# uniio/ivf-hnsw

Measured on AMD Instinct MI355X. Metric: queries/sec @ Recall@1, SIFT1B PQ16 nprobe=32; ADC scan HBM GB/s vs peak, higher is better.
Workload: dtype f32

## Files before the change

### ivf-hnsw_amd/csrc/device_common.h

```cpp
#pragma once
#include <hip/hip_runtime.h>
#include <stdint.h>

#include "scan_dispatch.h"

namespace ivfhnsw_gpu_impl {

__device__ __forceinline__ float l2_ref_order(const float *__restrict__ row, const float *sq, int d)
{
    float a0 = 0.f, a1 = 0.f, a2 = 0.f, a3 = 0.f, a4 = 0.f, a5 = 0.f, a6 = 0.f, a7 = 0.f;
    const float4 *r4 = reinterpret_cast<const float4 *>(row);
    const float4 *q4 = reinterpret_cast<const float4 *>(sq);
    for (int b = 0; b < d / 16; b++) {
        const float4 y0 = r4[4 * b], y1 = r4[4 * b + 1], y2 = r4[4 * b + 2], y3 = r4[4 * b + 3];
        const float4 x0 = q4[4 * b], x1 = q4[4 * b + 1], x2 = q4[4 * b + 2], x3 = q4[4 * b + 3];
        float t;
#define IVFHNSW_ACC(a, xv, yv) \
    t = __fsub_rn(xv, yv);     \
    a = __fadd_rn(a, __fmul_rn(t, t));
        IVFHNSW_ACC(a0, x0.x, y0.x) IVFHNSW_ACC(a1, x0.y, y0.y) IVFHNSW_ACC(a2, x0.z, y0.z) IVFHNSW_ACC(a3, x0.w, y0.w)
        IVFHNSW_ACC(a4, x1.x, y1.x) IVFHNSW_ACC(a5, x1.y, y1.y) IVFHNSW_ACC(a6, x1.z, y1.z) IVFHNSW_ACC(a7, x1.w, y1.w)
        IVFHNSW_ACC(a0, x2.x, y2.x) IVFHNSW_ACC(a1, x2.y, y2.y) IVFHNSW_ACC(a2, x2.z, y2.z) IVFHNSW_ACC(a3, x2.w, y2.w)
        IVFHNSW_ACC(a4, x3.x, y3.x) IVFHNSW_ACC(a5, x3.y, y3.y) IVFHNSW_ACC(a6, x3.z, y3.z) IVFHNSW_ACC(a7, x3.w, y3.w)
#undef IVFHNSW_ACC
// ... 126 lines not shown
        const float2 x = q2[4 * (j0 + i)];
        const float d0 = __fsub_rn(x.x, y[i].x), d1 = __fsub_rn(x.y, y[i].y);
        alo = __fadd_rn(alo, __fmul_rn(d0, d0));
        ahi = __fadd_rn(ahi, __fmul_rn(d1, d1));
    }
}

__device__ __forceinline__ float l2_ref_order_quad_batched(const float *row, const float *sq, int d, int t)
{
    const float2 *r2 = reinterpret_cast<const float2 *>(row) + t;
    const float2 *q2 = reinterpret_cast<const float2 *>(sq) + t;
    float alo = 0.f, ahi = 0.f;
    const int nj = d >> 3;
    int j0 = 0;
    for (; j0 + 16 <= nj; j0 += 16)
        l2_quad_block<16>(r2, q2, j0, alo, ahi);
    if (j0 + 8 <= nj) {
        l2_quad_block<8>(r2, q2, j0, alo, ahi);
        j0 += 8;
    }
    if (j0 + 4 <= nj) {
        l2_quad_block<4>(r2, q2, j0, alo, ahi);
        j0 += 4;
    }
    if (j0 + 2 <= nj)
        l2_quad_block<2>(r2, q2, j0, alo, ahi);
    float r = __fadd_rn(quad_bcast<0>(alo), quad_bcast<0>(ahi));
    r = __fadd_rn(r, quad_bcast<1>(alo));
    r = __fadd_rn(r, quad_bcast<1>(ahi));
    r = __fadd_rn(r, quad_bcast<2>(alo));
    r = __fadd_rn(r, quad_bcast<2>(ahi));
    r = __fadd_rn(r, quad_bcast<3>(alo));
    r = __fadd_rn(r, quad_bcast<3>(ahi));
    return r;
}

template <int NB>
__device__ __forceinline__ void l2_oct_block(const float *r1, const float *q1, int j0, float &acc)
{
    float y[NB];
#pragma unroll
    for (int i = 0; i < NB; i++)
        y[i] = r1[8 * (j0 + i)];
    asm volatile("" ::: "memory");
    __builtin_amdgcn_sched_barrier(0);
#pragma unroll
    for (int i = 0; i < NB; i++) {
        const float d0 = __fsub_rn(q1[8 * (j0 + i)], y[i]);
        acc = __fadd_rn(acc, __fmul_rn(d0, d0));
    }
}

__device__ __forceinline__ float l2_ref_order_oct(const float *row, const float *sq, int d, int t)
{
    const float *r1 = row + t;
    const float *q1 = sq + t;
    float acc = 0.f;
    const int nj = d >> 3;
    int j0 = 0;
    for (; j0 + 16 <= nj; j0 += 16)
        l2_oct_block<16>(r1, q1, j0, acc);
    if (j0 + 8 <= nj) {
        l2_oct_block<8>(r1, q1, j0, acc);
        j0 += 8;
    }
    if (j0 + 4 <= nj) {
        l2_oct_block<4>(r1, q1, j0, acc);
        j0 += 4;
    }
    if (j0 + 2 <= nj)
        l2_oct_block<2>(r1, q1, j0, acc);
    const float mir = __uint_as_float(
        (uint32_t)__builtin_amdgcn_update_dpp(0, (int)__float_as_uint(acc), 0x141, 0xf, 0xf, true));
    float r = __fadd_rn(quad_bcast<0>(acc), quad_bcast<1>(acc));
    r = __fadd_rn(r, quad_bcast<2>(acc));
    r = __fadd_rn(r, quad_bcast<3>(acc));
    r = __fadd_rn(r, quad_bcast<3>(mir));
    r = __fadd_rn(r, quad_bcast<2>(mir));
    r = __fadd_rn(r, quad_bcast<1>(mir));
    r = __fadd_rn(r, quad_bcast<0>(mir));
    return r;
}

template <int NJ>
__device__ __forceinline__ float l2_ref_order_oct_regs(const float *row, const float (&qr)[16], int t)
{
    const float *r1 = row + t;
    float y[NJ];
#pragma unroll
    for (int i = 0; i < NJ; i++)
        y[i] = r1[8 * i];
    asm volatile("" ::: "memory");
    __builtin_amdgcn_sched_barrier(0);
    float acc = 0.f;
#pragma unroll
    for (int i = 0; i < NJ; i++) {
        const float d0 = __fsub_rn(qr[i], y[i]);
        acc = __fadd_rn(acc, __fmul_rn(d0, d0));
    }
    const float mir = __uint_as_float(
        (uint32_t)__builtin_amdgcn_update_dpp(0, (int)__float_as_uint(acc), 0x141, 0xf, 0xf, true));
    float r = __fadd_rn(quad_bcast<0>(acc), quad_bcast<1>(acc));
    r = __fadd_rn(r, quad_bcast<2>(acc));
    r = __fadd_rn(r, quad_bcast<3>(acc));
    r = __fadd_rn(r, quad_bcast<3>(mir));
    r = __fadd_rn(r, quad_bcast<2>(mir));
    r = __fadd_rn(r, quad_bcast<1>(mir));
    r = __fadd_rn(r, quad_bcast<0>(mir));
    return r;
}

__device__ __forceinline__ float quad_sum8(float alo, float ahi)
{
    float r = __fadd_rn(quad_bcast<0>(alo), quad_bcast<0>(ahi));
    r = __fadd_rn(r, quad_bcast<1>(alo));
    r = __fadd_rn(r, quad_bcast<1>(ahi));
    r = __fadd_rn(r, quad_bcast<2>(alo));
    r = __fadd_rn(r, quad_bcast<2>(ahi));
    r = __fadd_rn(r, quad_bcast<3>(alo));
    r = __fadd_rn(r, quad_bcast<3>(ahi));
    return r;
}

__device__ __forceinline__ uint32_t wave_incl_scan(uint32_t v, int lane)
{
    (void)lane;
    int x = (int)v;
    x += __builtin_amdgcn_update_dpp(0, x, 0x111, 0xf, 0xf, true);
    x += __builtin_amdgcn_update_dpp(0, x, 0x112, 0xf, 0xf, true);
    x += __builtin_amdgcn_update_dpp(0, x, 0x114, 0xf, 0xf, true);
    x += __builtin_amdgcn_update_dpp(0, x, 0x118, 0xf, 0xf, true);
    x += __builtin_amdgcn_update_dpp(0, x, 0x142, 0xa, 0xf, false);
    x += __builtin_amdgcn_update_dpp(0, x, 0x143, 0xc, 0xf, false);
    return (uint32_t)x;
}

__device__ __forceinline__ unsigned long long wave_incl_scan_u64(unsigned long long v, int lane)
{
#pragma unroll
    for (int off = 1; off < 64; off <<= 1) {
        const unsigned long long o = __shfl_up(v, off, 64);
        if (lane >= off)
            v += o;
    }
    return v;
}

__device__ __forceinline__ uint64_t wave_min_u64(uint64_t v)
{
#pragma unroll
    for (int off = 32; off >= 1; off >>= 1) {
        uint64_t o = __shfl_xor((unsigned long long)v, off, 64);
        v = o < v ? o : v;
    }
    return v;
}

__device__ __forceinline__ uint32_t f32_orderable(float f)
{
    uint32_t u = __float_as_uint(f);
    return (u & 0x80000000u) ? ~u : (u | 0x80000000u);
}
__device__ __forceinline__ float orderable_f32(uint32_t o)
{
    return __uint_as_float((o & 0x80000000u) ? (o & 0x7fffffffu) : ~o);
}


template <int CS>
__device__ __forceinline__ void load_code_words(const uint8_t *__restrict__ codes, uint32_t gi, uint32_t (&w)[CS / 4])
{
    const uint8_t *p = codes + (size_t)gi * CS;
    if constexpr (CS % 16 == 0) {
#pragma unroll
        for (int i = 0; i < CS / 16; i++) {
            uint4 v = reinterpret_cast<const uint4 *>(p)[i];
            w[4 * i] = v.x, w[4 * i + 1] = v.y, w[4 * i + 2] = v.z, w[4 * i + 3] = v.w;
        }
    } else if constexpr (CS % 8 == 0) {
#pragma unroll
        for (int i = 0; i < CS / 8; i++) {
            uint2 v = reinterpret_cast<const uint2 *>(p)[i];
            w[2 * i] = v.x, w[2 * i + 1] = v.y;
        }
    } else {
#pragma unroll
        for (int i = 0; i < CS / 4; i++)
            w[i] = reinterpret_cast<const uint32_t *>(p)[i];
    }
}

template <int CS>
// ... 140 lines not shown
```

### ivf-hnsw_amd/csrc/kernels_hnsw.hip

```cpp
#include "ivfhnsw_kernels.h"
#include "device_common.h"
#include "walk_set.h"
#include "walk_shape.h"

#include <float.h>
#include <stdio.h>
#include <stdlib.h>
#include <type_traits>

namespace ivfhnsw_gpu_impl {

constexpr int vis_buckets(int minw, int tagw = 8)
{
    return minw <= 4 ? (tagw == 10 ? 1040 : 1008) : minw == 5 ? 768 : minw <= 7 ? 640 : 384;
}

template <int TAGW> struct VisFields {
    static constexpr int cntw = TAGW == 8 ? 8 : TAGW == 10 ? 14 : 16;
    static constexpr int cshift = 64 - cntw;
    static constexpr int slots = cshift / TAGW;
    static constexpr unsigned long long ones()
    {
        unsigned long long o = 0;
        for (int i = 0; i < slots; i++)
// ... 54 lines not shown
{
    static_assert(TAGW != 0, "LDS set only");
    constexpr unsigned long long kOnes = VisFields<TAGW>::ones();
    constexpr unsigned long long kHighs = kOnes << (TAGW - 1);
    const uint32_t b = id % (uint32_t)NB;
    const unsigned long long tag = (unsigned long long)((id / (uint32_t)NB) + 1);
    const unsigned long long old = vt[b];
    const unsigned long long x = old ^ (tag * kOnes);
    bucket_full = false;
    if ((x - kOnes) & ~x & kHighs)
        return true;
    bucket_full = (uint32_t)(old >> VisFields<TAGW>::cshift) >= (uint32_t)VisFields<TAGW>::slots;
    if (!bucket_full)
        return false;
    return (atomicOr(&bm[id >> 5], 0u) >> (id & 31)) & 1u;
}

__device__ __forceinline__ float byte_row_dist_half(const uint8_t *row, const float *sqp, int d, int h)
{
    const uint4 *r4 = reinterpret_cast<const uint4 *>(row);
    const int nchunk = d >> 4;
    float a0 = 0.f, a1 = 0.f, a2 = 0.f, a3 = 0.f;
    for (int j0 = h; j0 < nchunk; j0 += 8) {
        uint4 w[4];
#pragma unroll
        for (int i = 0; i < 4; i++)
            w[i] = j0 + 2 * i < nchunk ? r4[j0 + 2 * i] : make_uint4(0u, 0u, 0u, 0u);
        asm volatile("" ::: "memory");
        __builtin_amdgcn_sched_barrier(0);
#pragma unroll
        for (int i = 0; i < 4; i++) {
            if (j0 + 2 * i < nchunk) {
                const float4 *qq = reinterpret_cast<const float4 *>(sqp + 16 * (j0 + 2 * i));
                const uint32_t ws[4] = {w[i].x, w[i].y, w[i].z, w[i].w};
#pragma unroll
                for (int c = 0; c < 4; c++) {
                    const float4 qv = qq[c];
                    const float t0 = qv.x - (float)(ws[c] & 0xffu);
                    const float t1 = qv.y - (float)((ws[c] >> 8) & 0xffu);
                    const float t2 = qv.z - (float)((ws[c] >> 16) & 0xffu);
                    const float t3 = qv.w - (float)(ws[c] >> 24);
                    a0 = fmaf(t0, t0, a0);
                    a1 = fmaf(t1, t1, a1);
                    a2 = fmaf(t2, t2, a2);
                    a3 = fmaf(t3, t3, a3);
                }
            }
        }
    }
    return (a0 + a1) + (a2 + a3);
}

__device__ __forceinline__ unsigned long long walk_stamp()
{
    __builtin_amdgcn_sched_barrier(0);
    const unsigned long long t = __builtin_amdgcn_s_memtime();
    __builtin_amdgcn_s_waitcnt(0xC07F);
    __builtin_amdgcn_sched_barrier(0);
    return t;
}


struct WalkArgs {
    GraphTables g;
    const float *xq;
    int nq, nprobe, ef;
    uint32_t *coarse_ids;
    float *coarse_dists;
    uint32_t *visited;
    size_t vwords;
    uint32_t *status, *next_query, *redo_hdr, *redo_list;
    uint32_t *tail_bitmaps;
    unsigned long long *stamp_out;
};

template <class T> __device__ __forceinline__ const __attribute__((address_space(4))) T *late_kernarg()
{
    auto p = (const __attribute__((address_space(4))) T *)__builtin_amdgcn_kernarg_segment_ptr();
    asm volatile("" : "+s"(p));
    return p;
}

template <int NCH, int MINW, int TAGW, int FMODE, bool STAMPS = false, bool SPILL = false, int D = 0, int MAXM = 0,
          bool MERGE = true>
__global__ __launch_bounds__(64, MINW) void hnsw_walk_kernel(WalkArgs a)
{
    constexpr bool SHAPED = D != 0 && MAXM != 0;
    const GraphTables &g = a.g;
    const int ef = a.ef;
    uint32_t *__restrict__ const visited = a.visited;
    const size_t vwords = a.vwords;
#define WALK_COLD(f) (SHAPED ? late_kernarg<WalkArgs>()->f : a.f)
    extern __shared__ __attribute__((aligned(16))) unsigned char smem[];
    float *s_q = reinterpret_cast<float *>(smem);
    static_assert(!SHAPED || (FMODE >= 2 && !SPILL && MINW <= 4 && D % 16 == 0 && D <= 128 && MAXM <= 64),
                  "shape constants go with the neighbour-row forms");
    static_assert(SHAPED || MERGE, "the generic form reads merge_admissions at run time");
    const int dim = D ? D : g.d;
    const int maxm = MAXM ? MAXM : g.maxM;
    const int nbr_rows = MAXM ? (MAXM + 31) / 32 * 32 : g.nb_rows;
    float *s_qp = s_q + dim;
    const int dp = FMODE == 1 ? dim : 0;
    uint32_t *s_q8 = reinterpret_cast<uint32_t *>(s_qp + dp);
    unsigned long long *tail = reinterpret_cast<unsigned long long *>(smem + (size_t)(dim + dp) * sizeof(float) + 512);
    constexpr int NB = vis_buckets(MINW, TAGW);
    unsigned long long st_acc[9] = {0, 0, 0, 0, 0, 0}, st_t = 0;
    const int merge_extra = (NCH <= 4 && ef + 8 > kTailCap) ? ef + 8 - kTailCap : 0;
    unsigned long long *vt = tail + kTailCap + merge_extra;
    constexpr bool LDSVIS = TAGW != 0;

    const int lane = threadIdx.x;
    const int judged_row = 8 * (((lane >> 2) & 1) * 2 + (lane & 1)) + (lane >> 3);
    const bool merge_on = SHAPED ? MERGE : g.merge_admissions != 0;
    constexpr bool prefilter = FMODE != 0;
    constexpr bool inline_rows = FMODE >= 2;
    constexpr bool ROWNORMS = FMODE == 3;
    constexpr bool CK = FMODE >= 2;
    auto enc_id = [](uint32_t id, uint32_t c) { return CK ? (id << 7) | c : id; };
    auto dec_id = [](uint32_t e) { return CK ? e >> 7 : e; };
    uint32_t *bm = visited + (size_t)blockIdx.x * vwords;
    TailSpill spill;
    spill.bm = SPILL ? a.tail_bitmaps + (size_t)blockIdx.x * vwords : nullptr;
    spill.hi = -1;
    spill.count = 0;
    bool bitmap_dirty = !(LDSVIS && g.visited_clean);
    bool redo_ran = false;

    for (;;) {
        int q = 0;
        if constexpr (SPILL) {
            if (lane == 0) {
                const uint32_t i = atomicAdd(&a.redo_hdr[1], 1u);
                q = i < a.redo_hdr[0] ? (int)a.redo_list[i] : a.nq;
            }
        } else {
            if (lane == 0)
                q = (int)atomicAdd(WALK_COLD(next_query), 1u);
        }
        q = __builtin_amdgcn_readfirstlane(q);
        if (q >= WALK_COLD(nq))
            break;
        redo_ran = true;
        if (STAMPS)
            st_t = walk_stamp();

        if (!LDSVIS || bitmap_dirty) {
            uint4 *bm4 = reinterpret_cast<uint4 *>(bm);
            const size_t v4 = vwords / 4;
            for (size_t w = lane; w < v4; w += 64)
                bm4[w] = make_uint4(0u, 0u, 0u, 0u);
            bitmap_dirty = false;
        }
        if (LDSVIS)
            for (int w = lane; w < NB; w += 64)
                vt[w] = 0ull;
        __syncthreads();
        float qp_sq = 0.f;
        for (int i = lane; i < dim; i += 64) {
            const float v = WALK_COLD(xq)[(size_t)q * dim + i];
            s_q[i] = v;
            if (prefilter) {
                const float vp = __fdiv_rn(__fsub_rn(v, WALK_COLD(g.q_lo)), g.q_step);
                if (!inline_rows)
                    s_qp[i] = vp;
                qp_sq = fmaf(vp, vp, qp_sq);
            }
        }
        __syncthreads();
        constexpr bool QREG = MINW <= 4;
        float q_reg[QREG ? 16 : 1];
        if constexpr (QREG) {
#pragma unroll
            for (int i = 0; i < 16; i++)
                if constexpr (D != 0)
                    q_reg[i] = 8 * i < D ? s_q[8 * i + (lane & 7)] : 0.f;
                else
                    q_reg[i] = (g.d == 128 || g.d == 96) && 8 * i < g.d ? s_q[8 * i + (lane & 7)] : 0.f;
        }
        float pf_slack = 0.f, pf_slack_q = 0.f, pf_bonus = 0.f;
        int q16_w = 0;
        int x_const = 0;
        bool x_any = false;
        bool x_hi = false;
        uint4 qp_h = make_uint4(0u, 0u, 0u, 0u), qp_l = qp_h, qp_x = qp_h;
        if (prefilter) {
#pragma unroll
            for (int off = 32; off > 0; off >>= 1)
                qp_sq += __shfl_xor(qp_sq, off, 64);
            pf_slack = __uint_as_float(__builtin_amdgcn_readfirstlane(__float_as_uint(WALK_COLD(g.q_errc) + 3.9e-6f * sqrtf(qp_sq))));
// ... 254 lines not shown
                            if (x_hi) {
                                asm volatile("" ::);
#pragma unroll
                                for (int c = 0; c < 4; c++)
                                    xhr = __builtin_amdgcn_udot4(xh[c], ws[c], xhr, false);
                            }
                            X[i] = (int)(xlr - xhr);
                        }
                    }
                    int mine, minex = 0;
                    if (x_any)
                        oct_sum4x2(S, X, lane, mine, minex);
                    else
                        mine = oct_sum4(S, lane);
                    mine += (int)(128u * row_rr);
                    const float m1 = fmaxf(
                        0.f, __builtin_amdgcn_sqrtf((float)(mine + q16_w) * 0.0078125f) * 0.9990234375f - pf_slack_q);
                    const float m2 = fmaf(m1, m1, fmaf((float)(minex + x_const), 0.9990234375f, pf_bonus));
                    const float m = fmaxf(0.f, __builtin_amdgcn_sqrtf(m2) * 0.9990234375f - pf_slack) * g.q_step;
                    const float lb = m * m * 0.9990234375f;
                    const unsigned long long dropm = __ballot(lb > worst) & 0x3333333333333333ull;
                    const int rel = lane - rb;
                    const int ri = rel >> 3;
                    if (rel >= 0 && rel < 32 && ((dropm >> (8 * (rel & 7) + 4 * (ri >> 1) + (ri & 1))) & 1ull))
                        fresh = false;
                    rb += 32;
                    if (rb >= cnt)
                        break;
                    if constexpr (CK) {
                        const uint4 *nbr =
                            reinterpret_cast<const uint4 *>(g.nbrows + (size_t)node * nbr_rows * 128) + (lane & 7);
                        const int last = max(cnt - 1, 0);
#pragma unroll
                        for (int i = 0; i < 4; i++)
                            if (rb + 8 * i < cnt)
                                nw[i] = nbr[min(rb + 8 * i + (lane >> 3), last) * 8];
                    } else {
                        const uint4 *nbr =
                            reinterpret_cast<const uint4 *>(g.nbrows + ((size_t)node * nbr_rows + rb) * 128) + lane;
#pragma unroll
                        for (int i = 0; i < 4; i++)
                            nw[i] = nbr[i * 64];
                    }
                    if constexpr (ROWNORMS)
                        row_rr = g.nbnorms[(size_t)node * nbr_rows + rb + judged_row];
                }
                mask = __ballot(fresh);
                nfresh = __popcll(mask);
                if (filter_first) {
                    pend = fresh;
                    pend_full = full_now;
                    pend_id = nb;
                    pend_any = nfresh > 0;
                }
            } else if (filter_now && nfresh > 0) {
                const float worst = __uint_as_float(key_dist_bits(last_now));
                const int myrow = __popcll(mask & ((1ull << lane) - 1ull));
                for (int base = 0; base < nfresh; base += 32) {
                    const int r = base + (lane >> 1);
                    const bool active = r < nfresh;
                    const int src = active ? nth_set_bit(mask, r) : 0;
                    const uint32_t nbq = (uint32_t)__shfl((int)nb, src, 64);
                    float S = 0.f;
                    if (active)
                        S = byte_row_dist_half(g.qrows + (size_t)nbq * dim, s_qp, dim, lane & 1);
                    S += __shfl_xor(S, 1, 64);
                    const float m = fmaxf(0.f, __builtin_amdgcn_sqrtf(S) * 0.9990234375f - pf_slack) * g.q_step;
                    const float lb = m * m * 0.9990234375f;
                    const unsigned long long drop = __ballot(active && lb > worst);
                    const int rel = myrow - base;
                    if (fresh && rel >= 0 && rel < 32 && ((drop >> (2 * rel)) & 1ull))
                        fresh = false;
                }
                mask = __ballot(fresh);
                nfresh = __popcll(mask);
            }
            if (STAMPS) {
                const unsigned long long t = walk_stamp();
                st_acc[1] += t - st_t;
                st_t = t;
            }

            unsigned long long rest = mask;
            for (int base = 0; base < nfresh && ntail >= 0; base += 8) {
                const int r = base + (lane >> 3);
                const bool active = r < nfresh;
                const int src = take8_set_bits(rest, lane);
                const uint32_t nbe = (uint32_t)__shfl((int)nb_enc, src, 64);
                const uint32_t nbq = dec_id(nbe);
                float dq = 0.f;
                if (active) {
                    if constexpr (D != 0)
                        dq = l2_ref_order_oct_regs<D / 8>(g.vectors + (size_t)nbq * D, q_reg, lane & 7);
                    else if constexpr (QREG)
                        dq = g.d == 128  ? l2_ref_order_oct_regs<16>(g.vectors + (size_t)nbq * 128, q_reg, lane & 7)
                             : g.d == 96 ? l2_ref_order_oct_regs<12>(g.vectors + (size_t)nbq * 96, q_reg, lane & 7)
                                         : l2_ref_order_oct(g.vectors + (size_t)nbq * g.d, s_q, g.d, lane & 7);
                    else
                        dq = l2_ref_order_oct(g.vectors + (size_t)nbq * g.d, s_q, g.d, lane & 7);
                }
                if (STAMPS) {
                    asm volatile("s_waitcnt vmcnt(0)" ::: "memory");
                    const unsigned long long t = walk_stamp();
                    st_acc[2] += t - st_t;
                    st_t = t;
                }
                unsigned long long topk = base == 0 ? last_now : R.get(set_n() - 1);
                const float top0 = __uint_as_float(key_dist_bits(topk));
                unsigned long long cand = (!STEADY && n < ef ? ~0ull : __ballot(top0 > dq)) & 0x0101010101010101ull &
                                          lanes_below(8 * (nfresh - base), 0);
                if (STAMPS) {
                    st_acc[6] += (unsigned long long)__popcll(__ballot(active && (lane & 7) == 0));
                    st_acc[7] += (unsigned long long)__popcll(cand);
                }
                if (NCH <= 4 && merge_on && (STEADY || n == ef) && ntail == 0 && cand) {
                    const bool is_cand = (cand >> lane) & 1ull;
                    const unsigned long long Kc = mk_key(dq, nbe);
                    int dn[NCH];
#pragma unroll
                    for (int cc = 0; cc < NCH; cc++)
                        dn[cc] = 0;
                    const int ncand = __popcll(cand);
                    int cand_below = 0, set_below = 0;
                    for (unsigned long long cm = cand; cm; cm &= cm - 1) {
                        const int b = __ffsll((long long)cm) - 1;
                        const unsigned long long Kj = readlane_u64(Kc, b);
                        int below = 0;
#pragma unroll
                        for (int cc = 0; cc < NCH; cc++) {
                            const bool lt = (R.r[cc] & ~1ull) < Kj;
                            below += __popcll(__ballot(lt) & lanes_below(ef, cc));
                            dn[cc] += lt ? 1 : 0;
                        }
                        cand_below += Kj < Kc ? 1 : 0;
                        set_below = lane == b ? below : set_below;
                    }
                    unsigned long long *mb = tail;
#pragma unroll
                    for (int cc = 0; cc < NCH; cc++)
                        if (cc * 64 + lane < ef)
                            mb[cc * 64 + lane + (ncand - dn[cc])] = R.r[cc];
                    if (is_cand)
                        mb[set_below + cand_below] = Kc;
                    __syncthreads();
                    const unsigned long long b_lo = mb[ef - 1], b_hi = mb[ef];
                    unsigned long long merged[NCH];
#pragma unroll
                    for (int cc = 0; cc < NCH; cc++)
                        merged[cc] = cc * 64 + lane < ef ? mb[cc * 64 + lane] : R.r[cc];
                    const bool clean = key_dist_bits(b_lo) != key_dist_bits(b_hi);
                    if (clean) {
#pragma unroll
                        for (int cc = 0; cc < NCH; cc++)
                            R.r[cc] = merged[cc];
                        if (STAMPS)
                            st_acc[8] += (unsigned long long)__popcll(__ballot(is_cand && set_below + cand_below < ef));
                        cand = 0;
                    }
                    __syncthreads();
                }
                while (cand) {
                    const int b = __ffsll((long long)cand) - 1;
                    cand &= cand - 1;
                    const float dj = __uint_as_float((uint32_t)__builtin_amdgcn_readlane((int)__float_as_uint(dq), b));
                    const uint32_t idj = (uint32_t)__builtin_amdgcn_readlane((int)nbe, b);
                    const unsigned long long oldtop = topk;
                    if (!(__uint_as_float(key_dist_bits(oldtop)) > dj || (!STEADY && n < ef)))
                        continue;
                    const unsigned long long K = mk_key(dj, idj);
                    const bool full = STEADY || n == ef;
                    if (STAMPS)
                        st_acc[8] += 1;
                    R.insert_sorted(K, lane);
                    if (!full)
                        n++;
                    topk = R.get(set_n() - 1);
                    const uint32_t newmax = key_dist_bits(topk);
                    if (ntail > 0 && (SPILL ? tail_db : key_dist_bits(tail[0])) != newmax) {
                        ntail = 0;
                        if (SPILL && spill.count > 0)
                            spill.clear(lane);
                    }
                    if (full && !(oldtop & 1ull) && key_dist_bits(oldtop) == newmax) {
                        if (SPILL)
                            tail_db = newmax;
                        if ((!SPILL || spill.count == 0) && ntail < kTailCap) {
                            __syncthreads();
                            if (lane == 0)
                                tail[ntail] = oldtop;
                            ntail++;
                            __syncthreads();
                        } else if constexpr (SPILL) {
                            if (spill.count == 0) {
                                __syncthreads();
                                for (int t = 0; t < ntail; t++)
                                    spill.add(dec_id(key_id(tail[t])), lane);
                                __syncthreads();
                            }
                            spill.add(dec_id(key_id(oldtop)), lane);
                            ntail++;
                        } else {
                            if (lane == 0)
                                WALK_COLD(redo_list)[atomicAdd(&WALK_COLD(redo_hdr)[0], 1u)] = (uint32_t)q;
                            ntail = -1;
                            break;
                        }
                    }
                }
                if (STAMPS) {
                    const unsigned long long t = walk_stamp();
                    st_acc[3] += t - st_t;
                    st_t = t;
                }
            }
            return ntail >= 0;
        };
        if constexpr (SHAPED) {
            bool live = true;
            while (live && n < ef)
                live = expand(std::integral_constant<int, 1>{});
            while (live)
                live = expand(std::integral_constant<int, 2>{});
        } else {
            while (expand(std::integral_constant<int, 0>{})) {
            }
        }

        if (SPILL && spill.count > 0)
            spill.clear(lane);
        if (LDSVIS && __ballot(used_bitmap))
            bitmap_dirty = true;
        if (ntail >= 0) {
#pragma unroll
            for (int cc = 0; cc < NCH; cc++) {
                const int i = cc * 64 + lane;
                const int nprobe = WALK_COLD(nprobe);
                if (i < nprobe) {
                    const bool have = i < n;
                    WALK_COLD(coarse_ids)[(size_t)q * nprobe + i] = have ? dec_id(key_id(R.r[cc])) : 0xffffffffu;
                    WALK_COLD(coarse_dists)[(size_t)q * nprobe + i] = have ? __uint_as_float(key_dist_bits(R.r[cc])) : 0.f;
                }
            }
        }
    }
    if constexpr (SPILL) {
        if (lane == 0) {
            __threadfence();
            if (atomicAdd(&a.redo_hdr[2], 1u) == gridDim.x - 1) {
                a.redo_hdr[-1] = 0;
                a.redo_hdr[0] = 0;
                a.redo_hdr[1] = 0;
                a.redo_hdr[2] = 0;
            }
        }
    }
    if (SPILL && redo_ran) {
        uint4 *bm4 = reinterpret_cast<uint4 *>(bm);
        for (size_t w = lane; w < vwords / 4; w += 64)
            bm4[w] = make_uint4(0u, 0u, 0u, 0u);
    }
    if (LDSVIS && bitmap_dirty) {
        uint4 *bm4 = reinterpret_cast<uint4 *>(bm);
        for (size_t w = lane; w < vwords / 4; w += 64)
            bm4[w] = make_uint4(0u, 0u, 0u, 0u);
    }
    if (STAMPS && a.stamp_out && lane == 0)
        for (int i = 0; i < 9; i++)
            atomicAdd(&a.stamp_out[i], st_acc[i]);
#undef WALK_COLD
}

__global__ __launch_bounds__(64) void build_nbrows_kernel(GraphTables g, uint8_t *__restrict__ nbrows,
                                                          uint32_t *__restrict__ nbnorms, int nb_rows,
                                                          uint32_t *__restrict__ links_c)
{
    const size_t node = blockIdx.x;
    const int cnt = g.counts[node];
    if ((int)threadIdx.x < g.maxM) {
        uint32_t e = 0;
        if ((int)threadIdx.x < cnt) {
            const uint32_t id = g.links[node * g.maxM + threadIdx.x];
            e = id | ((uint32_t)g.counts[id] << 24);
        }
        links_c[node * g.maxM + threadIdx.x] = e;
    }
    const int cpr = g.d >> 4;
    for (int r0 = 0; r0 < nb_rows; r0 += 8) {
        const int r = r0 + (threadIdx.x >> 3), c = threadIdx.x & 7;
        uint4 v = make_uint4(0u, 0u, 0u, 0u);
        if (r < cnt && c < cpr)
            v = reinterpret_cast<const uint4 *>(g.qrows + (size_t)g.links[node * g.maxM + r] * g.d)[c];
        reinterpret_cast<uint4 *>(nbrows + (node * nb_rows + r) * 128)[c] = v;
        uint32_t rr = 0;
        rr = __builtin_amdgcn_udot4(v.x, v.x, rr, false);
        rr = __builtin_amdgcn_udot4(v.y, v.y, rr, false);
        rr = __builtin_amdgcn_udot4(v.z, v.z, rr, false);
        rr = __builtin_amdgcn_udot4(v.w, v.w, rr, false);
        rr = (uint32_t)oct_sum((int)rr);
        if (c == 0)
            nbnorms[node * nb_rows + r] = rr;
    }
}

hipError_t launch_build_nbrows(hipStream_t s, const GraphTables &g, uint8_t *nbrows, uint32_t *nbnorms, int nb_rows,
                               uint32_t *links_c)
{
    if (!g.qrows || g.d > 128 || (g.d & 15) || nb_rows < g.maxM || (nb_rows & 31) || g.n >= (1u << 24) || g.maxM > 64)
        return hipErrorInvalidValue;
    hipLaunchKernelGGL(build_nbrows_kernel, dim3(g.n), dim3(64), 0, s, g, nbrows, nbnorms, nb_rows, links_c);
    return hipGetLastError();
}

int coarse_slots_for(int ef)
{
    const int nch = (ef + 63) / 64;
    const int waves_per_simd = nch <= 8 ? 4 : 3;
    return 256 * 4 * waves_per_simd;
}

hipError_t launch_coarse(hipStream_t s, const GraphTables &g_in, const float *xq, int nq, int nprobe, int ef,
                         uint32_t *coarse_ids, float *coarse_dists, uint32_t *visited_scratch,
                         size_t visited_words_per_slot, int nslots, uint32_t *status, uint32_t *next_query,
                         size_t visited_bytes, bool *visited_zero, uint32_t *redo_list, uint32_t *tail_bitmaps,
                         int tail_slots, bool *counters_clean)
{
    if (nq == 0)
        return hipSuccess;
    GraphTables g = g_in;
    if (ef > 1024 || ef < 1 || nprobe > ef || g.maxM > 64 || g.n >= 0x80000000u || (visited_words_per_slot & 3) ||
        !redo_list || !tail_bitmaps || tail_slots < 1)
        return hipErrorInvalidValue;
    uint32_t *redo_hdr = next_query + 1;
    hipError_t e = hipSuccess;
    if (!counters_clean || !*counters_clean) {
        e = hipMemsetAsync(next_query, 0, 4 * sizeof(uint32_t), s);
        if (e != hipSuccess)
            return e;
    }
    if (counters_clean)
        *counters_clean = false;
    constexpr int occ = 4;
    const int nch = (ef + 63) / 64;
    const int occ_eff = 4;
    uint32_t nbk = (uint32_t)vis_buckets(occ_eff);
    static const bool force_bitmap = [] {
        const char *e = getenv("IVFHNSW_WALK_VIS");
        return e && e[0] == 'b';
    }();
    int tagw = force_bitmap ? 0 : g.n <= 255u * nbk ? 8 : g.n <= 4095u * nbk ? 12 : g.n <= 65535u * nbk ? 16 : 0;
    static const int force_tagw = [] {
        const char *e = getenv("IVFHNSW_WALK_TAGW");
        const int v = e ? atoi(e) : 0;
        return (v == 10 || v == 12 || v == 16) ? v : 0;
    }();
    if (tagw && force_tagw > tagw)
        tagw = force_tagw;
    if ((tagw == 12 || tagw == 10) && occ_eff == 4 && g.n <= 1023u * (uint32_t)vis_buckets(4, 10) && force_tagw != 12) {
        tagw = 10;
        nbk = (uint32_t)vis_buckets(4, 10);
    } else if (tagw == 10) {
        tagw = 12;
    }
    const size_t shm = (size_t)(g.d + ((g.qrows && !g.nbrows) ? g.d : 0)) * sizeof(float) + 512 +
                       (size_t)(kTailCap + ((ef <= 256 && ef + 8 > kTailCap) ? ef + 8 - kTailCap : 0)) *
                           sizeof(unsigned long long) +
                       (tagw ? (size_t)nbk * sizeof(unsigned long long) : 0);
    const int fmode = g.nbrows ? (g.links_unique && tagw ? 3 : 2) : g.qrows ? 1 : 0;
    g.visited_clean = 0;
    if (tagw && visited_zero) {
        if (!*visited_zero) {
            e = hipMemsetAsync(visited_scratch, 0, visited_bytes, s);
            if (e != hipSuccess)
                return e;
        }
        g.visited_clean = 1;
        *visited_zero = true;
    } else if (visited_zero) {
        *visited_zero = false;
    }
    WalkArgs wa = {g,      xq,         nq,       nprobe,    ef,      coarse_ids, coarse_dists, visited_scratch, visited_words_per_slot,
                   status, next_query, redo_hdr, redo_list, nullptr, nullptr};
#define IVFHNSW_WALK_F(N, W, T, F) hipLaunchKernelGGL((hnsw_walk_kernel<N, W, T, F>), dim3(nslots), dim3(64), shm, s, wa)
#define IVFHNSW_WALK_T(N, W, T)          \
    do {                                 \
        if (fmode == 3)                  \
            IVFHNSW_WALK_F(N, W, T, 3);  \
        else if (fmode == 2)             \
            IVFHNSW_WALK_F(N, W, T, 2);  \
        else if (fmode == 1)             \
            IVFHNSW_WALK_F(N, 4, T, 1);  \
        else                             \
            IVFHNSW_WALK_F(N, 4, T, 0);  \
    } while (0)
#define IVFHNSW_WALK(N, W)             \
    do {                               \
        if (tagw == 8)                 \
            IVFHNSW_WALK_T(N, W, 8);   \
        else if (tagw == 10)           \
            IVFHNSW_WALK_T(N, 4, 10);  \
        else if (tagw == 12)           \
            IVFHNSW_WALK_T(N, W, 12);  \
        else if (tagw == 16)           \
            IVFHNSW_WALK_T(N, W, 16);  \
        else                           \
            IVFHNSW_WALK_T(N, W, 0);   \
    } while (0)
#define IVFHNSW_WALK_N(N) IVFHNSW_WALK(N, 4)
    static const bool stamps = [] {
        const char *e = getenv("IVFHNSW_WALK_STAMPS");
        return e && atoi(e) == 1;
    }();
    static const bool shape_on = [] {
        const char *e = getenv("IVFHNSW_WALK_SHAPE");
        return !(e && atoi(e) == 0);
    }();
    const WalkShape shape = walk_shape_for(g.d, g.maxM, g.nb_rows, fmode, tagw, nch, shape_on);
    const bool merge = g.merge_admissions != 0;
    if (stamps && nch == 2 && ((tagw == 8 && fmode == 2) || (tagw == 10 && fmode == 3)) && occ == 4) {
        static unsigned long long *d_st = nullptr;
        if (!d_st) {
            (void)hipMalloc(&d_st, 9 * sizeof(unsigned long long));
            (void)hipMemset(d_st, 0, 9 * sizeof(unsigned long long));
            atexit([] {
                unsigned long long h[9];
                if (hipMemcpy(h, d_st, sizeof(h), hipMemcpyDeviceToHost) == hipSuccess) {
                    const double tot = (double)(h[0] + h[1] + h[2] + h[3] + h[4]);
                    fprintf(stderr, "[walk stamps] expansions %llu; cycles/expansion: select %.0f, links+visited %.0f, "
                                    "distances %.0f, admissions %.0f; prologue share %.1f%%; total wave-cycles %.3g\n",
                            h[5], (double)h[0] / h[5], (double)h[1] / h[5], (double)h[2] / h[5], (double)h[3] / h[5],
                            100.0 * h[4] / tot, tot);
                    fprintf(stderr, "[walk stamps] rows evaluated/expansion %.2f, passing the wave-wide test %.2f, admitted %.2f\n",
                            (double)h[6] / h[5], (double)h[7] / h[5], (double)h[8] / h[5]);
                }
            });
        }
        wa.stamp_out = d_st;
        if (tagw == 8)
            hipLaunchKernelGGL((hnsw_walk_kernel<2, 4, 8, 2, true>), dim3(nslots), dim3(64), shm, s, wa);
        else if (shape.d == 128 && merge)
            hipLaunchKernelGGL((hnsw_walk_kernel<2, 4, 10, 3, true, false, 128, 32, true>), dim3(nslots), dim3(64), shm, s, wa);
        else
            hipLaunchKernelGGL((hnsw_walk_kernel<2, 4, 10, 3, true>), dim3(nslots), dim3(64), shm, s, wa);
        return hipGetLastError();
    }
#define IVFHNSW_WALK_S(N, T, F, DD, MG) \
    hipLaunchKernelGGL((hnsw_walk_kernel<N, 4, T, F, false, false, DD, 32, MG>), dim3(nslots), dim3(64), shm, s, wa)
#define IVFHNSW_WALK_SD(N, T, F)                   \
    do {                                           \
        if (shape.d == 128 && merge)               \
            IVFHNSW_WALK_S(N, T, F, 128, true);    \
        else if (shape.d == 128)                   \
            IVFHNSW_WALK_S(N, T, F, 128, false);   \
        else if (merge)                            \
            IVFHNSW_WALK_S(N, T, F, 96, true);     \
        else                                       \
            IVFHNSW_WALK_S(N, T, F, 96, false);    \
    } while (0)
#define IVFHNSW_WALK_ST(N, T)            \
    do {                                 \
        if (fmode == 3)                  \
            IVFHNSW_WALK_SD(N, T, 3);    \
        else                             \
            IVFHNSW_WALK_SD(N, T, 2);    \
    } while (0)
#define IVFHNSW_WALK_SN(N)               \
    do {                                 \
        if (tagw == 8)                   \
            IVFHNSW_WALK_ST(N, 8);       \
        else if (tagw == 10)             \
            IVFHNSW_WALK_ST(N, 10);      \
        else if (tagw == 12)             \
            IVFHNSW_WALK_ST(N, 12);      \
        else                             \
            IVFHNSW_WALK_ST(N, 16);      \
    } while (0)
    if (shape.d != 0 && nch <= 1) {
        IVFHNSW_WALK_SN(1);
    } else if (shape.d != 0) {
        IVFHNSW_WALK_SN(2);
    } else
    if (nch <= 1) {
        IVFHNSW_WALK_N(1);
    } else if (nch <= 2) {
        IVFHNSW_WALK_N(2);
    } else if (nch == 3) {
        IVFHNSW_WALK_N(3);
    } else if (nch <= 4) {
        IVFHNSW_WALK_N(4);
    } else if (nch <= 8) {
        IVFHNSW_WALK(8, 4);
    } else {
        IVFHNSW_WALK(16, 4);
    }
#undef IVFHNSW_WALK_SN
#undef IVFHNSW_WALK_ST
#undef IVFHNSW_WALK_SD
#undef IVFHNSW_WALK_S
#undef IVFHNSW_WALK_N
#undef IVFHNSW_WALK
#undef IVFHNSW_WALK_T
#undef IVFHNSW_WALK_F
    e = hipGetLastError();
    if (e != hipSuccess)
        return e;
    e = launch_coarse_redo(s, g, xq, nq, nprobe, ef, coarse_ids, coarse_dists, visited_scratch, visited_words_per_slot,
                           status, redo_hdr, redo_list, tail_bitmaps, tail_slots);
    if (e == hipSuccess && counters_clean)
        *counters_clean = true;
    return e;
}

hipError_t launch_coarse_redo(hipStream_t s, const GraphTables &g_in, const float *xq, int nq, int nprobe, int ef,
                              uint32_t *coarse_ids, float *coarse_dists, uint32_t *visited_scratch,
                              size_t visited_words_per_slot, uint32_t *status, uint32_t *redo_hdr, uint32_t *redo_list,
                              uint32_t *tail_bitmaps, int tail_slots)
{
    GraphTables g = g_in;
    g.visited_clean = 0;
    const int nch = (ef + 63) / 64;
    const int slots = std::min(std::min(nq, tail_slots), 64);
    const size_t shm = (size_t)g.d * sizeof(float) + 512 +
                       (size_t)(kTailCap + ((ef <= 256 && ef + 8 > kTailCap) ? ef + 8 - kTailCap : 0)) * sizeof(unsigned long long);
    const WalkArgs wa = {g,      xq,           nq,       nprobe,    ef,           coarse_ids, coarse_dists, visited_scratch, visited_words_per_slot,
                         status, redo_hdr + 1, redo_hdr, redo_list, tail_bitmaps, nullptr};
#define IVFHNSW_REDO(N) hipLaunchKernelGGL((hnsw_walk_kernel<N, 4, 0, 0, false, true>), dim3(slots), dim3(64), shm, s, wa)
    if (nch <= 1)
        IVFHNSW_REDO(1);
    else if (nch <= 2)
        IVFHNSW_REDO(2);
// ... 14 lines not shown
```

Baseline: 6.549 million.

## Prefetch next pass of neighbour rows in HNSW walk and use wave-local LDS sync

In the shaped walk kernel, the neighbour-row loads for the next 8-row pass are issued before the current pass's admission and merge work, so global memory latency overlaps with that work. The change holds a full row (D/8 floats per lane) in registers across the loop, which raises register pressure. It also swaps the two __syncthreads around the LDS merge for a wave-only lgkmcnt wait plus wave barrier, which is valid because the block is a single 64-lane wave. The prefetch path is on by default and can be turned off with an environment variable. Stamp counters for passes per expansion are added.

Result: no change. 6.613 million (median of 6 runs) (+1.0%).

```diff
diff --git a/ivf-hnsw_amd/csrc/device_common.h b/ivf-hnsw_amd/csrc/device_common.h
--- a/ivf-hnsw_amd/csrc/device_common.h
+++ b/ivf-hnsw_amd/csrc/device_common.h
@@ -232,32 +232,52 @@
     return r;
 }
 
+template <int NJ> struct OctRow {
+    float y[NJ];
+};
+
+template <int NJ> __device__ __forceinline__ void oct_row_load(OctRow<NJ> &r, const float *row, int t)
+{
+    const float *r1 = row + t;
+#pragma unroll
+    for (int i = 0; i < NJ; i++)
+        r.y[i] = r1[8 * i];
+    asm volatile("" ::: "memory");
+    __builtin_amdgcn_sched_barrier(0);
+}
+
+template <int NJ> __device__ __forceinline__ float oct_row_dist(const OctRow<NJ> &r, const float (&qr)[16])
+{
+    float acc = 0.f;
+#pragma unroll
+    for (int i = 0; i < NJ; i++) {
+        const float d0 = __fsub_rn(qr[i], r.y[i]);
+        acc = __fadd_rn(acc, __fmul_rn(d0, d0));
+    }
+    const float mir = __uint_as_float(
+        (uint32_t)__builtin_amdgcn_update_dpp(0, (int)__float_as_uint(acc), 0x141, 0xf, 0xf, true));
+    float r0 = __fadd_rn(quad_bcast<0>(acc), quad_bcast<1>(acc));
+    r0 = __fadd_rn(r0, quad_bcast<2>(acc));
+    r0 = __fadd_rn(r0, quad_bcast<3>(acc));
+    r0 = __fadd_rn(r0, quad_bcast<3>(mir));
+    r0 = __fadd_rn(r0, quad_bcast<2>(mir));
+    r0 = __fadd_rn(r0, quad_bcast<1>(mir));
+    r0 = __fadd_rn(r0, quad_bcast<0>(mir));
+    return r0;
+}
+
 template <int NJ>
 __device__ __forceinline__ float l2_ref_order_oct_regs(const float *row, const float (&qr)[16], int t)
 {
-    const float *r1 = row + t;
-    float y[NJ];
-#pragma unroll
-    for (int i = 0; i < NJ; i++)
-        y[i] = r1[8 * i];
-    asm volatile("" ::: "memory");
-    __builtin_amdgcn_sched_barrier(0);
-    float acc = 0.f;
-#pragma unroll
-    for (int i = 0; i < NJ; i++) {
-        const float d0 = __fsub_rn(qr[i], y[i]);
-        acc = __fadd_rn(acc, __fmul_rn(d0, d0));
-    }
-    const float mir = __uint_as_float(
-        (uint32_t)__builtin_amdgcn_update_dpp(0, (int)__float_as_uint(acc), 0x141, 0xf, 0xf, true));
-    float r = __fadd_rn(quad_bcast<0>(acc), quad_bcast<1>(acc));
-    r = __fadd_rn(r, quad_bcast<2>(acc));
-    r = __fadd_rn(r, quad_bcast<3>(acc));
-    r = __fadd_rn(r, quad_bcast<3>(mir));
-    r = __fadd_rn(r, quad_bcast<2>(mir));
-    r = __fadd_rn(r, quad_bcast<1>(mir));
-    r = __fadd_rn(r, quad_bcast<0>(mir));
-    return r;
+    OctRow<NJ> r;
+    oct_row_load(r, row, t);
+    return oct_row_dist(r, qr);
+}
+
+__device__ __forceinline__ void wave_lds_sync()
+{
+    asm volatile("s_waitcnt lgkmcnt(0)" ::: "memory");
+    __builtin_amdgcn_wave_barrier();
 }
 
 __device__ __forceinline__ float quad_sum8(float alo, float ahi)
diff --git a/ivf-hnsw_amd/csrc/kernels_hnsw.hip b/ivf-hnsw_amd/csrc/kernels_hnsw.hip
--- a/ivf-hnsw_amd/csrc/kernels_hnsw.hip
+++ b/ivf-hnsw_amd/csrc/kernels_hnsw.hip
@@ -160,7 +160,7 @@
 }
 
 template <int NCH, int MINW, int TAGW, int FMODE, bool STAMPS = false, bool SPILL = false, int D = 0, int MAXM = 0,
-          bool MERGE = true>
+          bool MERGE = true, bool AHEAD = false>
 __global__ __launch_bounds__(64, MINW) void hnsw_walk_kernel(WalkArgs a)
 {
     constexpr bool SHAPED = D != 0 && MAXM != 0;
@@ -174,6 +174,7 @@
     static_assert(!SHAPED || (FMODE >= 2 && !SPILL && MINW <= 4 && D % 16 == 0 && D <= 128 && MAXM <= 64),
                   "shape constants go with the neighbour-row forms");
     static_assert(SHAPED || MERGE, "the generic form reads merge_admissions at run time");
+    static_assert(SHAPED || !AHEAD, "requesting a pass ahead goes with the shaped forms");
     const int dim = D ? D : g.d;
     const int maxm = MAXM ? MAXM : g.maxM;
     const int nbr_rows = MAXM ? (MAXM + 31) / 32 * 32 : g.nb_rows;
@@ -182,7 +183,7 @@
     uint32_t *s_q8 = reinterpret_cast<uint32_t *>(s_qp + dp);
     unsigned long long *tail = reinterpret_cast<unsigned long long *>(smem + (size_t)(dim + dp) * sizeof(float) + 512);
     constexpr int NB = vis_buckets(MINW, TAGW);
-    unsigned long long st_acc[9] = {0, 0, 0, 0, 0, 0}, st_t = 0;
+    unsigned long long st_acc[12] = {0, 0, 0, 0, 0, 0}, st_t = 0;
     const int merge_extra = (NCH <= 4 && ef + 8 > kTailCap) ? ef + 8 - kTailCap : 0;
     unsigned long long *vt = tail + kTailCap + merge_extra;
     constexpr bool LDSVIS = TAGW != 0;
@@ -603,28 +604,60 @@
             }
 
             unsigned long long rest = mask;
+            if (STAMPS) {
+                st_acc[9] += (unsigned long long)((nfresh + 7) >> 3);
+                st_acc[10] += nfresh > 8 ? 1 : 0;
+                st_acc[11] += nfresh > 16 ? 1 : 0;
+            }
+            OctRow<AHEAD ? D / 8 : 2> yrow;
+            uint32_t nbe_dealt = 0;
+            auto deal = [&](int base) __attribute__((always_inline)) {
+                if constexpr (AHEAD) {
+                    const int src = take8_set_bits(rest, lane);
+                    nbe_dealt = (uint32_t)__shfl((int)nb_enc, src, 64);
+                    if (base + (lane >> 3) < nfresh)
+                        oct_row_load(yrow, g.vectors + (size_t)dec_id(nbe_dealt) * D, lane & 7);
+                }
+            };
+            if constexpr (AHEAD)
+                if (nfresh > 0)
+                    deal(0);
             for (int base = 0; base < nfresh && ntail >= 0; base += 8) {
                 const int r = base + (lane >> 3);
                 const bool active = r < nfresh;
-                const int src = take8_set_bits(rest, lane);
-                const uint32_t nbe = (uint32_t)__shfl((int)nb_enc, src, 64);
-                const uint32_t nbq = dec_id(nbe);
+                uint32_t nbe;
                 float dq = 0.f;
-                if (active) {
-                    if constexpr (D != 0)
-                        dq = l2_ref_order_oct_regs<D / 8>(g.vectors + (size_t)nbq * D, q_reg, lane & 7);
-                    else if constexpr (QREG)
-                        dq = g.d == 128  ? l2_ref_order_oct_regs<16>(g.vectors + (size_t)nbq * 128, q_reg, lane & 7)
-                             : g.d == 96 ? l2_ref_order_oct_regs<12>(g.vectors + (size_t)nbq * 96, q_reg, lane & 7)
-                                         : l2_ref_order_oct(g.vectors + (size_t)nbq * g.d, s_q, g.d, lane & 7);
-                    else
-                        dq = l2_ref_order_oct(g.vectors + (size_t)nbq * g.d, s_q, g.d, lane & 7);
-                }
-                if (STAMPS) {
-                    asm volatile("s_waitcnt vmcnt(0)" ::: "memory");
-                    const unsigned long long t = walk_stamp();
-                    st_acc[2] += t - st_t;
-                    st_t = t;
+                if constexpr (AHEAD) {
+                    nbe = nbe_dealt;
+                    if (active)
+                        dq = oct_row_dist(yrow, q_reg);
+                    if (STAMPS) {
+                        const unsigned long long t = walk_stamp();
+                        st_acc[2] += t - st_t;
+                        st_t = t;
+                    }
+                    if (base + 8 < nfresh)
+                        deal(base + 8);
+                } else {
+                    const int src = take8_set_bits(rest, lane);
+                    nbe = (uint32_t)__shfl((int)nb_enc, src, 64);
+                    const uint32_t nbq = dec_id(nbe);
+                    if (active) {
+                        if constexpr (D != 0)
+                            dq = l2_ref_order_oct_regs<D / 8>(g.vectors + (size_t)nbq * D, q_reg, lane & 7);
+                        else if constexpr (QREG)
+                            dq = g.d == 128  ? l2_ref_order_oct_regs<16>(g.vectors + (size_t)nbq * 128, q_reg, lane & 7)
+                                 : g.d == 96 ? l2_ref_order_oct_regs<12>(g.vectors + (size_t)nbq * 96, q_reg, lane & 7)
+                                             : l2_ref_order_oct(g.vectors + (size_t)nbq * g.d, s_q, g.d, lane & 7);
+                        else
+                            dq = l2_ref_order_oct(g.vectors + (size_t)nbq * g.d, s_q, g.d, lane & 7);
+                    }
+                    if (STAMPS) {
+                        asm volatile("s_waitcnt vmcnt(0)" ::: "memory");
+                        const unsigned long long t = walk_stamp();
+                        st_acc[2] += t - st_t;
+                        st_t = t;
+                    }
                 }
                 unsigned long long topk = base == 0 ? last_now : R.get(set_n() - 1);
                 const float top0 = __uint_as_float(key_dist_bits(topk));
@@ -663,7 +696,7 @@
                             mb[cc * 64 + lane + (ncand - dn[cc])] = R.r[cc];
                     if (is_cand)
                         mb[set_below + cand_below] = Kc;
-                    __syncthreads();
+                    wave_lds_sync();
                     const unsigned long long b_lo = mb[ef - 1], b_hi = mb[ef];
                     unsigned long long merged[NCH];
 #pragma unroll
@@ -678,7 +711,7 @@
                             st_acc[8] += (unsigned long long)__popcll(__ballot(is_cand && set_below + cand_below < ef));
                         cand = 0;
                     }
-                    __syncthreads();
+                    wave_lds_sync();
                 }
                 while (cand) {
                     const int b = __ffsll((long long)cand) - 1;
@@ -786,7 +819,7 @@
             bm4[w] = make_uint4(0u, 0u, 0u, 0u);
     }
     if (STAMPS && a.stamp_out && lane == 0)
-        for (int i = 0; i < 9; i++)
+        for (int i = 0; i < 12; i++)
             atomicAdd(&a.stamp_out[i], st_acc[i]);
 #undef WALK_COLD
 }
@@ -936,14 +969,18 @@
         return !(e && atoi(e) == 0);
     }();
     const WalkShape shape = walk_shape_for(g.d, g.maxM, g.nb_rows, fmode, tagw, nch, shape_on);
+    static const bool ahead = [] {
+        const char *e = getenv("IVFHNSW_WALK_AHEAD");
+        return !(e && atoi(e) == 0);
+    }();
     const bool merge = g.merge_admissions != 0;
     if (stamps && nch == 2 && ((tagw == 8 && fmode == 2) || (tagw == 10 && fmode == 3)) && occ == 4) {
         static unsigned long long *d_st = nullptr;
         if (!d_st) {
-            (void)hipMalloc(&d_st, 9 * sizeof(unsigned long long));
-            (void)hipMemset(d_st, 0, 9 * sizeof(unsigned long long));
+            (void)hipMalloc(&d_st, 12 * sizeof(unsigned long long));
+            (void)hipMemset(d_st, 0, 12 * sizeof(unsigned long long));
             atexit([] {
-                unsigned long long h[9];
+                unsigned long long h[12];
                 if (hipMemcpy(h, d_st, sizeof(h), hipMemcpyDeviceToHost) == hipSuccess) {
                     const double tot = (double)(h[0] + h[1] + h[2] + h[3] + h[4]);
                     fprintf(stderr, "[walk stamps] expansions %llu; cycles/expansion: select %.0f, links+visited %.0f, "
@@ -952,20 +989,32 @@
                             100.0 * h[4] / tot, tot);
                     fprintf(stderr, "[walk stamps] rows evaluated/expansion %.2f, passing the wave-wide test %.2f, admitted %.2f\n",
                             (double)h[6] / h[5], (double)h[7] / h[5], (double)h[8] / h[5]);
+                    fprintf(stderr, "[walk stamps] passes/expansion %.3f; expansions with more than one pass %llu (%.2f%%), "
+                                    "with more than two %llu (%.2f%%)\n",
+                            (double)h[9] / h[5], h[10], 100.0 * h[10] / h[5], h[11], 100.0 * h[11] / h[5]);
                 }
             });
         }
         wa.stamp_out = d_st;
         if (tagw == 8)
             hipLaunchKernelGGL((hnsw_walk_kernel<2, 4, 8, 2, true>), dim3(nslots), dim3(64), shm, s, wa);
+        else if (shape.d == 128 && merge && ahead)
+            hipLaunchKernelGGL((hnsw_walk_kernel<2, 4, 10, 3, true, false, 128, 32, true, true>), dim3(nslots), dim3(64), shm, s, wa);
         else if (shape.d == 128 && merge)
             hipLaunchKernelGGL((hnsw_walk_kernel<2, 4, 10, 3, true, false, 128, 32, true>), dim3(nslots), dim3(64), shm, s, wa);
         else
             hipLaunchKernelGGL((hnsw_walk_kernel<2, 4, 10, 3, true>), dim3(nslots), dim3(64), shm, s, wa);
         return hipGetLastError();
     }
-#define IVFHNSW_WALK_S(N, T, F, DD, MG) \
-    hipLaunchKernelGGL((hnsw_walk_kernel<N, 4, T, F, false, false, DD, 32, MG>), dim3(nslots), dim3(64), shm, s, wa)
+#define IVFHNSW_WALK_S(N, T, F, DD, MG)                                                                                        \
+    do {                                                                                                                      \
+        if (ahead)                                                                                                            \
+            hipLaunchKernelGGL((hnsw_walk_kernel<N, 4, T, F, false, false, DD, 32, MG, true>), dim3(nslots), dim3(64), shm, s, \
+                               wa);                                                                                           \
+        else                                                                                                                  \
+            hipLaunchKernelGGL((hnsw_walk_kernel<N, 4, T, F, false, false, DD, 32, MG, false>), dim3(nslots), dim3(64), shm,  \
+                               s, wa);                                                                                        \
+    } while (0)
 #define IVFHNSW_WALK_SD(N, T, F)                   \
     do {                                           \
         if (shape.d == 128 && merge)               \
```
